# rdd0582/mri_superresolution

Measured on AMD Instinct MI355X. Metric: 2D MRI slices/sec (train fwd+bwd) 256×256 U-Net; PSNR/SSIM vs ref, higher is better.
Workload: dtype bf16; 1 GPU; UNetSuperRes base_filters=64 depth=4, 256x256 slices -> 512x512, batch=16/GPU bf16, L1+SSIM(0.4), train step fwd+bwd+Adam+SSIM metric; global_batch=16, parallelism=dp1

## Files before the change

mri_superresolution_amd/csrc/conv_pack.hip:

```cpp
#include "conv_common.h"
#include "conv_upadj.h"

template <typename T>
__global__ void pack_weights_kernel(const float* __restrict__ w, T* __restrict__ out, int Cout, int Cin,
                                    int KS, int flip, int BN, int ncb, int nchunks) {
    constexpr int BK = kRowBytes / (int)sizeof(T);
    const int ntaps = KS * KS;
    const size_t total = (size_t)ncb * nchunks * ntaps * BN * BK;
    const int Co = flip ? Cin : Cout, Ci = flip ? Cout : Cin;
    for (size_t idx = blockIdx.x * (size_t)blockDim.x + threadIdx.x; idx < total;
         idx += (size_t)gridDim.x * blockDim.x) {
        size_t r = idx;
        const int e = r % BK; r /= BK;
        const int row = r % BN; r /= BN;
        const int tap = r % ntaps; r /= ntaps;
        const int kc = r % nchunks;
        const int cb = r / nchunks;
        constexpr int EPC = 16 / (int)sizeof(T);
        const int q = tap * BN + row;
        const int chunk_pos = e / EPC, chunk = chunk_pos ^ ((q >> 2) & 3);
        const int k = kc * BK + chunk * EPC + (e % EPC);
        const int co = cb * BN + row;
        float v = 0.f;
        if (co < Co && k < Ci) {
            if (!flip) v = w[((size_t)co * ntaps + tap) * Cin + k];
            else v = w[((size_t)k * ntaps + (ntaps - 1 - tap)) * Cin + co];
        }
        out[idx] = from_f32<T>(v);
    }
}

struct PackJobDev { const float* w; void* packed; int Cout, Cin, ksize, flip; };
template <typename T>
__global__ void pack_weights_batched_kernel(const PackJobDev* __restrict__ jobs) {
    constexpr int BK = kRowBytes / (int)sizeof(T);
    constexpr int EPC = 16 / (int)sizeof(T);
    const PackJobDev j = jobs[blockIdx.y];
    const int KS = j.ksize, ntaps = KS * KS, Cin = j.Cin, Cout = j.Cout, flip = j.flip & 1;
    const int Co = flip ? Cin : Cout, Ci = flip ? Cout : Cin;
    const float* __restrict__ w = j.w;
    auto gather = [&](int co, int tap, int k0, Vec16<T>& v) {
#pragma unroll
        for (int e = 0; e < EPC; ++e) {
            const int k = k0 + e;
            float x = 0.f;
            if (co < Co && k < Ci) x = !flip ? w[((size_t)co * ntaps + tap) * Cin + k] : w[((size_t)k * ntaps + (ntaps - 1 - tap)) * Cin + co];
            v.set(e, x);
        }
    };
    if (j.flip & MRISR_PACK_UPADJ) {
        if (!conv_upadj_image_bytes(TypeTraits<T>::kDtype, Cout, Cin, KS)) return;
        const int RS = upadj_rs(Cout), K9 = ntaps * Cout;
        const size_t nchunk = (size_t)Cin * RS / EPC;
        for (size_t idx = blockIdx.x * (size_t)blockDim.x + threadIdx.x; idx < nchunk; idx += (size_t)gridDim.x * blockDim.x) {
            const int ci = (int)(idx * EPC / RS), k0 = (int)(idx * EPC % RS);
            Vec16<T> v;
#pragma unroll
            for (int e = 0; e < EPC; ++e) {
                const int k = k0 + e;
                v.set(e, k < K9 ? w[((size_t)(k % Cout) * ntaps + k / Cout) * Cin + ci] : 0.f);
            }
            store_vec16((T*)j.packed + idx * EPC, v);
        }
        return;
    }
    if (j.flip & MRISR_PACK_RING) {
        const int RBN = conv_ring_bn(TypeTraits<T>::kDtype, Co, Ci, KS);
        if (RBN == 0) return;
        const int rnch = Ci / 16;
        const size_t nchunk = (size_t)(Co / RBN) * rnch * ntaps * RBN * 2;
        for (size_t idx = blockIdx.x * (size_t)blockDim.x + threadIdx.x; idx < nchunk; idx += (size_t)gridDim.x * blockDim.x) {
            size_t r = idx;
            const int pos = r & 1; r >>= 1;
            const int row = r % RBN; r /= RBN;
            const int tap = r % ntaps; r /= ntaps;
            const int kc = r % rnch;
            const int cb = r / rnch;
            const int slot = pos ^ ((row >> 3) & 1);
            Vec16<T> v;
            gather(cb * RBN + row, tap, kc * 16 + slot * 8, v);
            store_vec16((T*)j.packed + idx * EPC, v);
        }
        return;
    }
    const int BN = Co >= 64 ? 64 : 32;
    const int ncb = (Co + BN - 1) / BN, nchunks = (Ci + BK - 1) / BK;
    const size_t nchunk = (size_t)ncb * nchunks * ntaps * BN * 4;
    for (size_t idx = blockIdx.x * (size_t)blockDim.x + threadIdx.x; idx < nchunk; idx += (size_t)gridDim.x * blockDim.x) {
        size_t r = idx;
        const int pos = r & 3; r >>= 2;
        const int row = r % BN; r /= BN;
        const int tap = r % ntaps; r /= ntaps;
        const int kc = r % nchunks;
        const int cb = r / nchunks;
        const int q = tap * BN + row;
        const int chunk = pos ^ ((q >> 2) & 3);
        Vec16<T> v;
        gather(cb * BN + row, tap, kc * BK + chunk * EPC, v);
        store_vec16((T*)j.packed + idx * EPC, v);
    }
}

extern "C" int mrisr_pack_weights_batched(int dtype, const mrisr_pack_job* jobs_device, int njobs, void* stream) {
    static_assert(sizeof(PackJobDev) == sizeof(mrisr_pack_job), "mrisr_pack_job layout");
    if (!jobs_device || njobs <= 0 || njobs > 65535) MRISR_FAIL(MRISR_E_ARG, "pack_weights_batched: bad job table");
    dim3 grid(256, njobs);
    if (dtype == MRISR_BF16)
        pack_weights_batched_kernel<bf16_t><<<grid, 256, 0, (hipStream_t)stream>>>((const PackJobDev*)jobs_device);
    else if (dtype == MRISR_F16)
        pack_weights_batched_kernel<f16_t><<<grid, 256, 0, (hipStream_t)stream>>>((const PackJobDev*)jobs_device);
    else if (dtype == MRISR_F32)
        pack_weights_batched_kernel<float><<<grid, 256, 0, (hipStream_t)stream>>>((const PackJobDev*)jobs_device);
    else
        MRISR_FAIL(MRISR_E_DTYPE, "pack_weights_batched: dtype %d", dtype);
    MRISR_CHECK_LAUNCH("pack_weights_batched");
    return MRISR_OK;
}

extern "C" size_t mrisr_packed_weight_bytes(int dtype, int Cout, int Cin, int ksize) {
    const int BN = conv_choose_bn(Cout), BK = conv_bk(dtype);
    const size_t ncb = ceil_div(Cout, BN), nch = ceil_div(Cin, BK);
    return ncb * nch * (size_t)(ksize * ksize) * BN * kRowBytes;
}

extern "C" int mrisr_pack_weights(int dtype, const float* w, int Cout, int Cin, int ksize, int transpose_flip,
                                  void* packed, void* stream) {
    if (!w || !packed) MRISR_FAIL(MRISR_E_ARG, "pack_weights: null pointer");
    if (ksize != 1 && ksize != 3) MRISR_FAIL(MRISR_E_UNSUPPORTED, "pack_weights: ksize %d", ksize);
    if (transpose_flip & (MRISR_PACK_RING | MRISR_PACK_UPADJ)) {
        const int flip = transpose_flip & 1;
        if ((transpose_flip & MRISR_PACK_UPADJ) && !conv_upadj_image_bytes(dtype, Cout, Cin, ksize))
            MRISR_FAIL(MRISR_E_UNSUPPORTED, "pack_weights: no upadj layout for %d -> %d k%d dtype %d", Cin, Cout, ksize, dtype);
        if (!(transpose_flip & MRISR_PACK_UPADJ) && !mrisr_conv_ring_bn(dtype, flip ? Cin : Cout, flip ? Cout : Cin, ksize))
            MRISR_FAIL(MRISR_E_UNSUPPORTED, "pack_weights: no ring layout for %d -> %d k%d dtype %d", Cin, Cout, ksize, dtype);
        const PackJobDev job{w, packed, Cout, Cin, ksize, transpose_flip};
        PackJobDev* dj = nullptr;
        if (hipMalloc(&dj, sizeof(job)) != hipSuccess) MRISR_FAIL(MRISR_E_HIP, "pack_weights: hipMalloc");
        (void)hipMemcpyAsync(dj, &job, sizeof(job), hipMemcpyHostToDevice, (hipStream_t)stream);
        const int rc = mrisr_pack_weights_batched(dtype, (const mrisr_pack_job*)dj, 1, stream);
        (void)hipStreamSynchronize((hipStream_t)stream);
        (void)hipFree(dj);
        return rc;
    }
    transpose_flip &= 1;
    const int Co = transpose_flip ? Cin : Cout, Ci = transpose_flip ? Cout : Cin;
    const int BN = conv_choose_bn(Co), BK = conv_bk(dtype);
    const int ncb = ceil_div(Co, BN), nch = ceil_div(Ci, BK);
    const size_t total = (size_t)ncb * nch * ksize * ksize * BN * BK;
    const int blocks = (int)((total + 255) / 256 < 4096 ? (total + 255) / 256 : 4096);
    if (dtype == MRISR_BF16)
        pack_weights_kernel<bf16_t><<<blocks, 256, 0, (hipStream_t)stream>>>(w, (bf16_t*)packed, Cout, Cin, ksize,
                                                                            transpose_flip, BN, ncb, nch);
    else if (dtype == MRISR_F16)
        pack_weights_kernel<f16_t><<<blocks, 256, 0, (hipStream_t)stream>>>(w, (f16_t*)packed, Cout, Cin, ksize,
                                                                           transpose_flip, BN, ncb, nch);
    else if (dtype == MRISR_F32)
        pack_weights_kernel<float><<<blocks, 256, 0, (hipStream_t)stream>>>(w, (float*)packed, Cout, Cin, ksize,
                                                                           transpose_flip, BN, ncb, nch);
    else
        MRISR_FAIL(MRISR_E_DTYPE, "pack_weights: dtype %d", dtype);
    MRISR_CHECK_LAUNCH("pack_weights");
    return MRISR_OK;
}
```

Baseline: 2109 slices/s.

## Load-balance batched weight packing across jobs and transpose tiles through LDS

The batched weight-pack kernel now builds an in-block prefix sum of per-job tile counts, so a fixed 2048-block grid spreads work evenly over all jobs instead of launching a 256×njobs grid. It also stages each weight tile in shared memory: coalesced reads from the fp32 weights go into LDS, and then 16-byte swizzled chunks are written out. This targets the scattered gathers, which are especially bad for the transposed/flipped layouts. The cost is extra __syncthreads per tile and a serial per-block walk over tiles. Packing runs once per optimizer step, so its share of the train step is small.

```diff
diff --git a/mri_superresolution_amd/csrc/conv_pack.hip b/mri_superresolution_amd/csrc/conv_pack.hip
--- a/mri_superresolution_amd/csrc/conv_pack.hip
+++ b/mri_superresolution_amd/csrc/conv_pack.hip
@@ -31,88 +31,133 @@
 }
 
 struct PackJobDev { const float* w; void* packed; int Cout, Cin, ksize, flip; };
+constexpr int kPackJobsPerLaunch = 256;
+constexpr int kPackBlocks = 2048;
+constexpr int kPackTilePad = 4;
+constexpr int kPackTileFloats = 128 * (16 + kPackTilePad);
+
 template <typename T>
-__global__ void pack_weights_batched_kernel(const PackJobDev* __restrict__ jobs) {
+__device__ __forceinline__ int pack_job_tiles(const PackJobDev& j) {
+    constexpr int BK = kRowBytes / (int)sizeof(T), EPC = 16 / (int)sizeof(T);
+    const int ntaps = j.ksize * j.ksize, flip = j.flip & 1;
+    const int Co = flip ? j.Cin : j.Cout, Ci = flip ? j.Cout : j.Cin;
+    if (j.flip & MRISR_PACK_UPADJ) {
+        if (!conv_upadj_image_bytes(TypeTraits<T>::kDtype, j.Cout, j.Cin, j.ksize)) return 0;
+        return (int)(((size_t)j.Cin * upadj_rs(j.Cout) / EPC + 255) / 256);
+    }
+    if (j.flip & MRISR_PACK_RING) {
+        const int RBN = conv_ring_bn(TypeTraits<T>::kDtype, Co, Ci, j.ksize);
+        return RBN ? (Co / RBN) * (Ci / 16) * ntaps : 0;
+    }
+    const int BN = Co >= 64 ? 64 : 32;
+    return ((Co + BN - 1) / BN) * ((Ci + BK - 1) / BK) * ntaps;
+}
+
+template <typename T>
+__global__ __launch_bounds__(256) void pack_weights_batched_kernel(const PackJobDev* __restrict__ jobs, int njobs) {
     constexpr int BK = kRowBytes / (int)sizeof(T);
     constexpr int EPC = 16 / (int)sizeof(T);
-    const PackJobDev j = jobs[blockIdx.y];
-    const int KS = j.ksize, ntaps = KS * KS, Cin = j.Cin, Cout = j.Cout, flip = j.flip & 1;
-    const int Co = flip ? Cin : Cout, Ci = flip ? Cout : Cin;
-    const float* __restrict__ w = j.w;
-    auto gather = [&](int co, int tap, int k0, Vec16<T>& v) {
-#pragma unroll
-        for (int e = 0; e < EPC; ++e) {
-            const int k = k0 + e;
-            float x = 0.f;
-            if (co < Co && k < Ci) x = !flip ? w[((size_t)co * ntaps + tap) * Cin + k] : w[((size_t)k * ntaps + (ntaps - 1 - tap)) * Cin + co];
-            v.set(e, x);
+    __shared__ int pre[kPackJobsPerLaunch + 1];
+    __shared__ int wave_tiles[4];
+    __shared__ __attribute__((aligned(16))) float tile_lds[kPackTileFloats];
+    const int t = threadIdx.x, lane = t & 63, wave = t >> 6;
+    int inc = t < njobs ? pack_job_tiles<T>(jobs[t]) : 0;
+#pragma unroll
+    for (int o = 1; o < 64; o <<= 1) {
+        const int v = __shfl_up(inc, o, 64);
+        if (lane >= o) inc += v;
+    }
+    if (lane == 63) wave_tiles[wave] = inc;
+    __syncthreads();
+    for (int wv = 0; wv < wave; ++wv) inc += wave_tiles[wv];
+    pre[t + 1] = inc;
+    if (t == 0) pre[0] = 0;
+    __syncthreads();
+    const int total = pre[kPackJobsPerLaunch];
+    const int share = (total + (int)gridDim.x - 1) / (int)gridDim.x;
+    int tile = blockIdx.x * share;
+    const int tend = min(total, tile + share);
+    if (tile >= tend) return;
+    int job = 0;
+#pragma unroll
+    for (int s = kPackJobsPerLaunch / 2; s > 0; s >>= 1)
+        if (pre[job + s] <= tile) job += s;
+    while (tile < tend) {
+        while (pre[job + 1] <= tile) ++job;
+        const PackJobDev j = jobs[job];
+        const int first = pre[job], jend = min(tend, pre[job + 1]);
+        const int KS = j.ksize, ntaps = KS * KS, Cin = j.Cin, Cout = j.Cout, flip = j.flip & 1;
+        const int Co = flip ? Cin : Cout, Ci = flip ? Cout : Cin;
+        const float* __restrict__ w = j.w;
+        if (j.flip & MRISR_PACK_UPADJ) {
+            const int RS = upadj_rs(Cout), K9 = ntaps * Cout;
+            const size_t nchunk = (size_t)Cin * RS / EPC;
+            for (; tile < jend; ++tile) {
+                const size_t idx = (size_t)(tile - first) * 256 + t;
+                if (idx >= nchunk) continue;
+                const int ci = (int)(idx * EPC / RS), k0 = (int)(idx * EPC % RS);
+                Vec16<T> v;
+#pragma unroll
+                for (int e = 0; e < EPC; ++e) {
+                    const int k = k0 + e;
+                    v.set(e, k < K9 ? w[((size_t)(k % Cout) * ntaps + k / Cout) * Cin + ci] : 0.f);
+                }
+                store_vec16((T*)j.packed + idx * EPC, v);
+            }
+            continue;
         }
-    };
-    if (j.flip & MRISR_PACK_UPADJ) {
-        if (!conv_upadj_image_bytes(TypeTraits<T>::kDtype, Cout, Cin, KS)) return;
-        const int RS = upadj_rs(Cout), K9 = ntaps * Cout;
-        const size_t nchunk = (size_t)Cin * RS / EPC;
-        for (size_t idx = blockIdx.x * (size_t)blockDim.x + threadIdx.x; idx < nchunk; idx += (size_t)gridDim.x * blockDim.x) {
-            const int ci = (int)(idx * EPC / RS), k0 = (int)(idx * EPC % RS);
-            Vec16<T> v;
-#pragma unroll
-            for (int e = 0; e < EPC; ++e) {
-                const int k = k0 + e;
-                v.set(e, k < K9 ? w[((size_t)(k % Cout) * ntaps + k / Cout) * Cin + ci] : 0.f);
-            }
-            store_vec16((T*)j.packed + idx * EPC, v);
+        const bool ring = (j.flip & MRISR_PACK_RING) != 0;
+        const int R = ring ? conv_ring_bn(TypeTraits<T>::kDtype, Co, Ci, KS) : (Co >= 64 ? 64 : 32);
+        const int KE = ring ? 16 : BK, stride = KE + kPackTilePad;
+        const int nch = ring ? Ci / 16 : (Ci + BK - 1) / BK;
+        const int r_sh = 31 - __clz(R), ke_sh = ring ? 4 : 31 - __clz(BK), cpr_sh = 31 - __clz(KE / EPC);
+        const int nelem = R * KE, nchk = nelem / EPC;
+        for (; tile < jend; ++tile) {
+            const int lt = tile - first;
+            const int tap = lt % ntaps, kc = (lt / ntaps) % nch, cb = (lt / ntaps) / nch;
+            float x[8];
+#pragma unroll
+            for (int u = 0; u < 8; ++u) {
+                const int i = t + u * 256;
+                const int row = flip ? i & (R - 1) : i >> ke_sh, k = flip ? i >> r_sh : i & (KE - 1);
+                const int co = cb * R + row, kk = kc * KE + k;
+                x[u] = 0.f;
+                if (i < nelem && co < Co && kk < Ci)
+                    x[u] = !flip ? w[((size_t)co * ntaps + tap) * Cin + kk] : w[((size_t)kk * ntaps + (ntaps - 1 - tap)) * Cin + co];
+            }
+            __syncthreads();
+#pragma unroll
+            for (int u = 0; u < 8; ++u) {
+                const int i = t + u * 256;
+                const int row = flip ? i & (R - 1) : i >> ke_sh, k = flip ? i >> r_sh : i & (KE - 1);
+                if (i < nelem) tile_lds[row * stride + k] = x[u];
+            }
+            __syncthreads();
+            if (t < nchk) {
+                const int row = t >> cpr_sh, pos = t & ((1 << cpr_sh) - 1);
+                const int chunk = ring ? pos ^ ((row >> 3) & 1) : pos ^ (((tap * R + row) >> 2) & 3);
+                const float* src = tile_lds + row * stride + chunk * EPC;
+                Vec16<T> v;
+#pragma unroll
+                for (int e = 0; e < EPC; ++e) v.set(e, src[e]);
+                store_vec16((T*)j.packed + ((size_t)lt * nchk + t) * EPC, v);
+            }
         }
-        return;
-    }
-    if (j.flip & MRISR_PACK_RING) {
-        const int RBN = conv_ring_bn(TypeTraits<T>::kDtype, Co, Ci, KS);
-        if (RBN == 0) return;
-        const int rnch = Ci / 16;
-        const size_t nchunk = (size_t)(Co / RBN) * rnch * ntaps * RBN * 2;
-        for (size_t idx = blockIdx.x * (size_t)blockDim.x + threadIdx.x; idx < nchunk; idx += (size_t)gridDim.x * blockDim.x) {
-            size_t r = idx;
-            const int pos = r & 1; r >>= 1;
-            const int row = r % RBN; r /= RBN;
-            const int tap = r % ntaps; r /= ntaps;
-            const int kc = r % rnch;
-            const int cb = r / rnch;
-            const int slot = pos ^ ((row >> 3) & 1);
-            Vec16<T> v;
-            gather(cb * RBN + row, tap, kc * 16 + slot * 8, v);
-            store_vec16((T*)j.packed + idx * EPC, v);
-        }
-        return;
-    }
-    const int BN = Co >= 64 ? 64 : 32;
-    const int ncb = (Co + BN - 1) / BN, nchunks = (Ci + BK - 1) / BK;
-    const size_t nchunk = (size_t)ncb * nchunks * ntaps * BN * 4;
-    for (size_t idx = blockIdx.x * (size_t)blockDim.x + threadIdx.x; idx < nchunk; idx += (size_t)gridDim.x * blockDim.x) {
-        size_t r = idx;
-        const int pos = r & 3; r >>= 2;
-        const int row = r % BN; r /= BN;
-        const int tap = r % ntaps; r /= ntaps;
-        const int kc = r % nchunks;
-        const int cb = r / nchunks;
-        const int q = tap * BN + row;
-        const int chunk = pos ^ ((q >> 2) & 3);
-        Vec16<T> v;
-        gather(cb * BN + row, tap, kc * BK + chunk * EPC, v);
-        store_vec16((T*)j.packed + idx * EPC, v);
     }
 }
 
 extern "C" int mrisr_pack_weights_batched(int dtype, const mrisr_pack_job* jobs_device, int njobs, void* stream) {
     static_assert(sizeof(PackJobDev) == sizeof(mrisr_pack_job), "mrisr_pack_job layout");
     if (!jobs_device || njobs <= 0 || njobs > 65535) MRISR_FAIL(MRISR_E_ARG, "pack_weights_batched: bad job table");
-    dim3 grid(256, njobs);
-    if (dtype == MRISR_BF16)
-        pack_weights_batched_kernel<bf16_t><<<grid, 256, 0, (hipStream_t)stream>>>((const PackJobDev*)jobs_device);
-    else if (dtype == MRISR_F16)
-        pack_weights_batched_kernel<f16_t><<<grid, 256, 0, (hipStream_t)stream>>>((const PackJobDev*)jobs_device);
-    else if (dtype == MRISR_F32)
-        pack_weights_batched_kernel<float><<<grid, 256, 0, (hipStream_t)stream>>>((const PackJobDev*)jobs_device);
-    else
-        MRISR_FAIL(MRISR_E_DTYPE, "pack_weights_batched: dtype %d", dtype);
+    if (!mrisr_dtype_ok(dtype)) MRISR_FAIL(MRISR_E_DTYPE, "pack_weights_batched: dtype %d", dtype);
+    for (int j0 = 0; j0 < njobs; j0 += kPackJobsPerLaunch) {
+        const PackJobDev* jd = (const PackJobDev*)jobs_device + j0;
+        const int n = njobs - j0 < kPackJobsPerLaunch ? njobs - j0 : kPackJobsPerLaunch;
+        with_dtype(dtype, [&](auto tag) {
+            using T = typename decltype(tag)::type;
+            pack_weights_batched_kernel<T><<<kPackBlocks, 256, 0, (hipStream_t)stream>>>(jd, n);
+        });
+    }
     MRISR_CHECK_LAUNCH("pack_weights_batched");
     return MRISR_OK;
 }
```

After: 2109 slices/s (median of 3 runs). Within noise of the previous version (+0.0%).
